# abacusorg/zeldovich-PLT

Hardware: AMD Instinct MI355X
Metric: particles/sec (grid->displacements) (higher is better)
Workload: dtype f64

## Files before the change

### zeldovich_plt_amd/api.py

```python
import ctypes as C
import os

import numpy as np

_HERE = os.path.dirname(os.path.abspath(__file__))
LIB_PATH = os.environ.get("ZD_LIB_PATH") or os.path.join(_HERE, "csrc", "build", "libzeldovich_hip.so")

ICFORMATS = {"Zeldovich": 0, "RVZel": 1, "RVdoubleZel": 2, "ZelSimple": 3}
RECORD_DTYPES = {
    "Zeldovich": np.dtype([("ijk", "<u2", 3), ("pad", "<u2"), ("d", "<f8", 3)]),
    "RVZel": np.dtype([("ijk", "<u2", 3), ("pad", "<u2"), ("d", "<f4", 3), ("v", "<f4", 3)]),
    "RVdoubleZel": np.dtype([("ijk", "<u2", 3), ("pad", "<u2"), ("d", "<f8", 3), ("v", "<f8", 3)]),
    "ZelSimple": np.dtype([("d", "<f4", 3)]),
}
KERNEL_NAMES = ("k_gen", "k_zfft", "k_yfft", "k_xfft", "z_stage", "exchange_wait")


class ZdParams(C.Structure):
    _fields_ = [
        ("ppd", C.c_int64), ("numblock", C.c_int32), ("cpd", C.c_int32), ("boxsize", C.c_double),
        ("fundamental", C.c_double), ("nyquist", C.c_double), ("k_cutoff", C.c_double),
        ("f_cluster", C.c_double), ("z_initial", C.c_double), ("PLT_target_z", C.c_double),
        ("seed", C.c_int64), ("corner_modes", C.c_int32), ("qdensity", C.c_int32),
        ("qoneslab", C.c_int32), ("qonemode", C.c_int32), ("one_mode", C.c_int32 * 3),
# ... 47 lines not shown
PASS_CB = C.CFUNCTYPE(C.c_int, C.c_void_p, C.c_int, C.c_int64, C.c_int64, C.c_void_p, C.c_void_p)
PARTICLE_CB = C.CFUNCTYPE(C.c_int, C.c_void_p, C.c_int64, C.c_int64, C.c_void_p)

EXPORTED_SYMBOLS = [
    "zd_generate", "zd_choose_stream_factor", "zd_plan_create", "zd_plan_destroy", "zd_plan_narray", "zd_plan_store_mode",
    "zd_plan_stream_factor", "zd_plan_passes", "zd_plan_plane_step", "zd_plan_record_size", "zd_plan_exchange_bytes", "zd_plan_local_planes",
    "zd_plan_plane_z", "zd_plan_stage_z", "zd_plan_stage_y", "zd_plan_stage_x", "zd_plan_stats", "zd_comm_unique_id", "zd_comm_create", "zd_comm_destroy", "zd_plan_ring_bytes", "zd_plan_run_pass",
    "zd_params_from_file", "zd_pk_create_from_file", "zd_pk_create_powerlaw", "zd_pk_power",
    "zd_pk_sigmaR", "zd_pk_destroy", "zd_load_eigmodes", "zd_free", "zd_comm_abort", "zd_comm_traffic", "zd_choose_pass_groups", "zd_plan_run_passes", "zd_comm_probe", "zd_choose_pass_groups_measured",
    "zd_dispatch_report", "zd_power_nbins", "zd_plan_measure_power", "zd_measure_power",
    "zd_plan_direct_sum", "zd_direct_sum", "zd_make_eigenmodes", "zd_write_eigmodes", "zd_param_file_string",
    "zd_plan_lpt_direct_sum", "zd_lpt_direct_sum", "zd_plan_lpt_power", "zd_lpt_power",
    "zd_interp_create", "zd_interp_add_plane", "zd_interp_result", "zd_interp_destroy", "zd_plan_interp", "zd_displace",
]
TESTING_SYMBOLS = ["zd_test_draws", "zd_test_modes", "zd_test_modes_table", "zd_test_v1_words", "zd_test_generate_loopback", "zd_test_fail_rank",
                   "zd_test_fft", "zd_test_ycols", "zd_test_poison", "zd_test_route", "zd_test_route_kernels", "zd_test_lpt2_coefficients", "zd_test_live_handles", "zd_test_plt_matrix"]
STORE_MODES = {"auto": 0, "reference": 1, "packed": 2, "fields": 3}

_lib = None
_testing_lib = None
TESTING_LIB_PATH = os.environ.get("ZD_TESTING_LIB_PATH") or os.path.join(_HERE, "csrc", "build", "libzeldovich_hip_testing.so")


def load_library():
    global _lib
    if _lib is None:
        _lib = _load(LIB_PATH, testing=False)
    return _lib


def load_testing_library():
# ... 13 lines not shown
    except ImportError:
        pass
    L = C.CDLL(path)
    vp, i32, i64, dbl = C.c_void_p, C.c_int32, C.c_int64, C.c_double
    L.zd_generate.argtypes = [C.POINTER(ZdParams), C.POINTER(ZdPk), vp, i64, SLAB_CB, vp, C.POINTER(ZdStats)]
    if testing:
        L.zd_test_generate_loopback.argtypes = L.zd_generate.argtypes
        L.zd_test_draws.argtypes = [i64, i64, vp, vp]
        L.zd_test_modes.argtypes = [C.POINTER(ZdParams), C.POINTER(ZdPk), i64, vp, vp]
        L.zd_test_modes_table.argtypes = [C.POINTER(ZdParams), C.POINTER(ZdPk), i64, vp, vp]
        L.zd_test_v1_words.argtypes = [i64, C.c_int32, vp]
        L.zd_test_fft.argtypes = [i32, i64, i32, vp, vp]
        L.zd_test_ycols.argtypes = [i32, i32, i32, i32, i32, vp, vp]
        L.zd_test_poison.argtypes = [C.c_int]
        L.zd_test_poison.restype = None
        L.zd_test_lpt2_coefficients.argtypes = [C.POINTER(ZdParams), vp]
        L.zd_test_lpt2_coefficients.restype = None
        L.zd_test_live_handles.argtypes = []
        L.zd_test_live_handles.restype = i64
        L.zd_test_plt_matrix.argtypes = [i64, dbl, i32, i64, vp, vp]
        L.zd_test_route_kernels.argtypes = [C.POINTER(ZdParams), i32, i32, i32, C.c_char_p, i64]
    L.zd_choose_stream_factor.argtypes = [C.POINTER(ZdParams), C.c_int, i64]
    L.zd_choose_pass_groups.argtypes = [C.POINTER(ZdParams), C.c_int, i64, C.POINTER(i32), C.POINTER(i32)]
    L.zd_plan_create.argtypes = [C.POINTER(ZdParams), C.POINTER(ZdPk), vp, i64, C.c_int, C.c_int, C.POINTER(vp)]
    L.zd_plan_destroy.argtypes = [vp]
    L.zd_plan_destroy.restype = None
    for name in ("zd_plan_narray", "zd_plan_store_mode", "zd_plan_stream_factor", "zd_plan_record_size", "zd_plan_passes", "zd_plan_plane_step"):
        getattr(L, name).argtypes = [vp]
        getattr(L, name).restype = i32
    for name in ("zd_plan_exchange_bytes", "zd_plan_local_planes"):
# ... 670 lines not shown
```

### zeldovich_plt_amd/csrc/zd_capi.cpp

```cpp
#include <hip/hip_runtime.h>

#include <atomic>
#include <chrono>
#include <condition_variable>
#include <deque>
#include <functional>
#include <mutex>
#include <new>
#include <thread>
#include <cmath>
#include <cstdio>
#include <cstdlib>
#include <cstring>
#include <vector>

#include "../../include/zeldovich_hip.h"
#include "zd_device.h"
#include "zd_launch.h"
#include "zd_plan.h"
#include "zd_glass.h"
#include "zd_route.h"
#include "zd_plt.h"
#ifdef ZD_TUNING
#include "zd_tuning.h"
// ... 46 lines not shown
            line[n - 1] = '\n';
        }
        if (buf && w == need && w + n < cap) {
            memcpy(buf + w, line, (size_t) n);
            w += n;
        }
        need += n;
    }
    if (buf && cap > 0) buf[w] = 0;
    return need + 1;
}

#ifdef ZD_TESTING
static std::atomic<int> g_poison{0};
void zd_test_poison(int on) { g_poison.store(on); }
#endif
hipError_t zd_store_alloc(void **p, size_t bytes) {
    hipError_t e = hipMalloc(p, bytes);
#ifdef ZD_TESTING
    if (e == hipSuccess && g_poison.load()) e = hipMemset(*p, 0xFF, bytes);
#endif
    return e;
}

namespace {

std::vector<cplx> make_twiddles(int n) {
    std::vector<cplx> tw(n);
    for (int k = 0; k < n; k++) {
        const long double a = 2.0L * 3.14159265358979323846264338327950288L * (long double) k / (long double) n;
// ... 921 lines not shown
                lBk = a; lBz = b; S.rows_outer = o;
            }
        }
        const int max_lBk = S.lHq + 1;
        while (lBk > max_lBk) lBk--;
        while ((1 << lBz) > pl->Zq) lBz--;
        S.lBk = lBk;
        S.lBz = lBz;
        S.one_block = (pl->nranks == 1 && lBk == S.lHq + 1 && lBz == 0 && !S.rows_outer) ? 1 : 0;
        int row_pad = store_row_pad(pl->N);
        if (const char *env = tune_env("ZD_PAD")) sscanf(env, "%d", &row_pad);
        pl->fused_z = pl->pack == zd::PACK_PLT3 && p->store_mode == ZD_STORE_AUTO && S.one_block && zd::genz_plt_supported(pl->N, pl->L)
                      && g.genf_tab && !v1 && p->qoneslab < 0 && main && p->k_cutoff >= 1.0
                      && (g.kmax == pl->half || !p->corner_modes) && (S.prune & 7) == 7 && !tune_env("ZD_NO_FUSED_Z");
        S.lq         = pl->fused_z ? 2 : 0;
        if (S.lq && !tune_env("ZD_PAD")) row_pad = store_row_pad(pl->N) / 2;
        S.pitch      = (pl->N + row_pad) << S.lq;
        S.a_rows     = (1 << lBk) << lBz;
        S.zb_rows    = S.a_rows * pl->narray;
        S.kb_rows    = S.zb_rows * ((pl->Zq >> S.lq) >> lBz);
        S.chunk_rows = S.kb_rows * ((2 * pl->Hq) >> lBk);
    }

    pl->ec.N        = pl->N;
    pl->ec.narray   = pl->narray;
    pl->ec.icformat = p->icformat;
    pl->ec.recsize  = record_size(p->icformat);
    pl->ec.qPLT     = p->qPLT;
    pl->ec.qdensity = p->qdensity;
    pl->ec.vnorm    = (p->qPLT || p->q2LPT) ? 1.0 : (sqrt(1. + 24 * p->f_cluster) - 1) * .25;
// ... 66 lines not shown
    zd::StoreLayout &S = pl->S;
    std::vector<zd::FieldRow> rows;
    const int64_t fe = field_rows(&pl->p, pl->nranks, &rows);
    HIPCHECK(upload(pl->d_fieldrows, rows));
    pl->F.lG          = S.lG;
    pl->F.lZq         = 0;
    while ((1 << pl->F.lZq) < pl->Zq) pl->F.lZq++;
    pl->F.Zq          = pl->Zq;
    pl->F.field_elems = fe;
    pl->F.ndens       = pl->dens ? 2 : 0;
    pl->F.nfield      = pl->pack == zd::PACK_PLTFIELD ? 6 : 4 + pl->F.ndens;
    pl->F.chunk_elems = (int64_t) pl->Zq * pl->F.nfield * fe;
    pl->F.rows        = pl->d_fieldrows;
    pl->store_bytes_  = pl->F.chunk_elems * pl->nranks * 16;
    pl->ring_planes = field_ring_planes(pl->N, pl->Zq);
    zd::StoreLayout &Q = pl->SR;
    Q            = S;
    Q.lq         = 0;
    Q.Hq         = pl->half;
    Q.lHq        = 0;
    while ((1 << Q.lHq) < pl->half) Q.lHq++;
    Q.lG         = 0;
    Q.ky_stride  = 1;
    Q.narray     = 3;
    Q.lBk        = Q.lHq + 1;
    Q.lBz        = 0;
    Q.rows_outer = 0;
    Q.one_block  = 1;
    Q.prune      = 0;
    Q.pitch      = pl->N + store_row_pad(pl->N);
// ... 1164 lines not shown
    zd::StoreLayout S;
    S.N = n; S.half = n / 2; S.Hq = n / 2; S.narray = narray;
    S.lHq = 0;
    while ((1 << S.lHq) < S.Hq) S.lHq++;
    S.lG = 0;
    S.ky_stride = 1;
    int lBk = 0, lBz = 0;
    if (tiled) {
        const long long target = std::max<long long>(1, ((long long) 2 << 20) / ((long long) n * 16));
        int lt = 0;
        while ((1LL << (lt + 1)) <= target) lt++;
        lBk = (lt + 1) / 2; lBz = lt - lBk;
        while ((1 << lBz) > nplanes) lBz--;
    }
    S.lq = 0;
    S.lBk = lBk; S.lBz = lBz; S.rows_outer = 0; S.one_block = 0; S.pitch = n; S.prune = 0; S.nt = 0; S.kmax = 0; S.fund2 = 0; S.k2_cutoff = 0;
    S.a_rows = (1 << lBk) << lBz;
    S.zb_rows = S.a_rows * narray;
    S.kb_rows = S.zb_rows * (nplanes >> lBz);
    S.chunk_rows = S.kb_rows * (n >> lBk);
    const size_t nel = (size_t) S.chunk_rows * S.pitch;
    DevBuf<cplx> d_tw, d;
    if (upload(d_tw, make_twiddles(n)) != hipSuccess || d.alloc(nel) != hipSuccess || hipMemset(d, 0, nel * sizeof(cplx)) != hipSuccess) return 1;
    float ms = 0;
    if (time_launches(reps, [&] { return zd::launch_yfft_variant(variant, S, nplanes, d_tw, d, 0); }, &ms)) return 1;
    *ms_per_launch = ms / reps;
    return 0;
}

int zd_test_copy_bw(int64_t bytes, int32_t reps, double *gbps) {
// ... 12 lines not shown
```

### zeldovich_plt_amd/csrc/zd_device.h

```cpp
#pragma once
#include <stdint.h>
#include "zd_fft.h"
#include "zd_pcg.h"
#if !defined(__HIPCC__)
struct double2 { double x, y; };
#endif

#ifdef ZD_TUNING
#define ZD_TUNE(x) ((x) != 0)
#else
#define ZD_TUNE(x) (false)
#endif

namespace zd {

constexpr int PK_LUT = 2048;

struct GenConst {
    int N, half;
    int kmax;
    int corner_modes;
    int qonemode, one_mode[3];
    int ablate;
    double fundamental, fundamental2, k2_cutoff;
// ... 55 lines not shown

struct StoreLayout {
    int N, half, Hq, narray;
    int lHq;
    int lG;
    int ky_stride;
    int lBk, lBz;
    int rows_outer;
    int one_block;
    int pitch;
    int chunk_rows, kb_rows, zb_rows, a_rows;
    int prune, kmax;
    double fund2, k2_cutoff;
    int nt;
    int lq;
};

constexpr int PRUNE_YTILE = 1 << 15;

ZD_HD bool column_is_zero(const StoreLayout &L, int kx, int ky) {
    if (!L.prune) return false;
    const int ax = kx < 0 ? -kx : kx, ay = ky < 0 ? -ky : ky;
    if (ax == L.kmax || ay == L.kmax) return true;
    return L.k2_cutoff > 0 && (double) (kx * kx + ky * ky) * L.fund2 >= L.k2_cutoff;
}

ZD_HD void row_slot(const StoreLayout &L, int ky, int &chunk, int &slot) {
    int kyh, tw;
    if (ky < L.half) {
        kyh = ky;
        tw  = 0;
// ... 104 lines not shown
ZD_HD void any_chunk_row(const AnyChunks &C, int y, int &chunk, int &slot) {
    const int half = C.N / 2;
    const int h = y < half ? y : (y == half ? 0 : C.N - y), tw = y < half ? 0 : 1;
    chunk = h & (C.G - 1);
    slot  = h / C.G + tw * C.Hq;
}

constexpr int NSLOT = 64;
struct Reduce {
    double sumsq[NSLOT];
    unsigned long long maxabs[3][NSLOT];
    unsigned long long maxkey[3][NSLOT];
    unsigned int lock[NSLOT];
};

template <int NT, int W>
__device__ __forceinline__ void ytile_of(int id, int &tile, int &a) {
    constexpr int TPL = W >= 8 ? 1 : 8 / W, GS = 6 * TPL;
    if constexpr (NT % (16 * TPL) == 0) {
        const int xcd = id & 7, s = id >> 3;
        const int g = (s / GS) * 8 + xcd, m = s % GS;
        const int side = m / (3 * TPL), mm = m % (3 * TPL);
        a    = mm / TPL;
        tile = side ? NT - 1 - (TPL * g + mm % TPL) : TPL * g + mm % TPL;
    } else {
        tile = id % NT;
        a    = id / NT;
    }
}

#if defined(__HIPCC__)
__device__ __forceinline__ bool mode_is_zero(const GenConst &g, int kx, int ky, int kz, double k2) {
    const int ax = kx < 0 ? -kx : kx, ay = ky < 0 ? -ky : ky, az = kz < 0 ? -kz : kz;
    if (ax == g.kmax || az == g.kmax || ay == g.kmax) return true;
// ... 8 lines not shown
```

### zeldovich_plt_amd/csrc/zd_kernels.hip

```cpp
#include <hip/hip_runtime.h>
#include <type_traits>
#include <stdint.h>
#include <stdio.h>
#include <algorithm>
#include <type_traits>
#include <stdlib.h>

#include "zd_device.h"
#include "zd_epi.h"
#include "zd_launch.h"
#include "zd_genmath.h"

using namespace zd;
using zdfft::cplx;
using zdpcg::u128;
using namespace zdgen;

__constant__ zdpcg::BitTable c_bits;

typedef double zd_d2v __attribute__((ext_vector_type(2)));
__device__ __forceinline__ cplx ld_stream(const cplx *p, bool nt) {
    if (nt) {
        const zd_d2v q = __builtin_nontemporal_load(reinterpret_cast<const zd_d2v *>(p));
        return cplx{q.x, q.y};
// ... 1204 lines not shown
    zdfft::fft_line<PL, LDS>(re, im, t, w, lds, twL);
    const FieldRow row = F.rows[kyloc0 / FIELD_RB + grp];
    const unsigned pos = ((unsigned) (x < row.split ? x : x - row.gap)) * FIELD_RB + r;
    const int Zq = 1 << F.lZq;
    int t2 = t;
    asm volatile("" : "+v"(t2));
#pragma unroll
    for (int e = 0; e < E; e++) {
        const int z2  = t2 + T * e;
        const int dst = z2 >> F.lZq, zl = z2 & (Zq - 1);
        out[(long long) dst * F.chunk_elems + (long long) (zl * F.nfield + (int) blockIdx.z) * F.field_elems + (unsigned) row.base + pos]
            = cplx{re[e], im[e]};
    }
}

template <int N, int E, int W, bool TWO>
__device__ __forceinline__ void yfft_f_unit_t(const FieldLayout &F, const StoreLayout &S, const cplx *__restrict__ tw,
                                              const cplx *__restrict__ store, int plane0, int ring_pitch, cplx *__restrict__ ring,
                                              int tile, int a, int pz, int unit, int t, int w, double *lds);

template <int N, int E, int W>
__device__ __forceinline__ void yfft_f_unit(const FieldLayout &F, const StoreLayout &S, const cplx *__restrict__ tw,
                                            const cplx *__restrict__ store, int plane0, int ring_pitch, cplx *__restrict__ ring,
                                            int id, int pz, int t, int w, double *lds) {
    using PL  = zdfft::Plan<N, E>;
    using LDS = zdfft::ColsInner<N, W>;
    constexpr int T = PL::T;
    constexpr int NT = N / W;
    int tile, a;
    ytile_of<NT, W>(id, tile, a);
    const int unit = pz * 3 * NT + id;
    if (F.nfield == 6 || a == 2)
        yfft_f_unit_t<N, E, W, true>(F, S, tw, store, plane0, ring_pitch, ring, tile, a, pz, unit, t, w, lds);
    else
        yfft_f_unit_t<N, E, W, false>(F, S, tw, store, plane0, ring_pitch, ring, tile, a, pz, unit, t, w, lds);
}

template <int N, int E, int W, bool TWO>
__device__ __forceinline__ void yfft_f_unit_t(const FieldLayout &F, const StoreLayout &S, const cplx *__restrict__ tw,
                                              const cplx *__restrict__ store, int plane0, int ring_pitch, cplx *__restrict__ ring,
                                              int tile, int a, int pz, [[maybe_unused]] int unit, int t, int w, double *lds) {
    using PL  = zdfft::Plan<N, E>;
    using LDS = zdfft::ColsInner<N, W>;
    constexpr int T = PL::T;
    const int x = tile * W + w, xm = (N - x) & (N - 1);
    const int zl = plane0 + pz;
#ifdef ZD_STAMPS
    if (zd_stamps && threadIdx.x == 0) {
        zd_stamps[(size_t) unit * 8 + 6] = __builtin_amdgcn_s_memrealtime();
        zd_stamps[(size_t) unit * 8 + 7] = (unsigned long long) __builtin_amdgcn_s_getreg((4 << 0) | (0 << 6) | (31 << 11))
                                           | ((unsigned long long) __builtin_amdgcn_s_getreg((20 << 0) | (0 << 6) | (31 << 11)) << 32);
    }
#endif
    ZD_STAMP(0, unit, false);
    const int kx = x > N / 2 ? x - N : x;
    if ((S.prune & PRUNE_YTILE) && __syncthreads_and(column_is_zero(S, kx, 0))) return;
    const bool plt = F.nfield == 6;
    constexpr bool two = TWO;
    const int f0 = plt ? (a == 0 ? 0 : (a == 1 ? 1 : 4)) : (a == 2 ? 1 : 2 * a);
    const int f1 = plt ? (a == 0 ? 3 : (a == 1 ? 2 : 5)) : 3;
    const cplx *p0 = store + (long long) (zl * F.nfield + f0) * F.field_elems;
    const long long d01 = two ? (long long) (f1 - f0) * F.field_elems : 0;
    const int gmask = (1 << F.lG) - 1;
    double re[E], im[E];
    FieldRow *rtab = reinterpret_cast<FieldRow *>(lds + LDS::SIZE);
    const int nblk = (S.Hq + FIELD_RB - 1) / FIELD_RB;
    for (int i = threadIdx.x; i < nblk; i += W * T) rtab[i] = F.rows[i];
    zdfft::TwSet<PL> twp;
    zdfft::load_twiddles<PL>(twp, t, tw);
    unsigned skipm = 1u << ((N / 2 - t) / T);
    if (t != 0) skipm = 0;
    if (S.prune & 4) {
        int c2 = 0x7fffffff;
        if (S.k2_cutoff > 0) {
            int m = (int) (S.k2_cutoff / S.fund2);
            while (m > 0 && (double) m * S.fund2 >= S.k2_cutoff) m--;
            while ((double) m * S.fund2 < S.k2_cutoff) m++;
            c2 = m;
        }
        const int akx = kx < 0 ? -kx : kx, kx2 = kx * kx;
#pragma unroll
        for (int e = 0; e < E; e++) {
            const int y = t + T * e, kyp = y > N / 2 ? N - y : y;
            if (akx == S.kmax || kyp == S.kmax || kx2 + kyp * kyp >= c2) skipm |= 1u << e;
        }
    }
// ... 27 lines not shown
        const cplx *p1 = p0 + d01;
#pragma unroll
        for (int b = 0; b < E; b += HB) {
            cplx v[HB];
            int tb = t;
            asm volatile("" : "+v"(tb));
#pragma unroll
            for (int j = 0; j < HB; j++) v[j] = p1[locate(tb, b + j)];
            asm volatile("" : "+v"(tb));
#pragma unroll
            for (int j = 0; j < HB; j++) {
                const int e = b + j, y = tb + T * e;
                const double s = y > N / 2 ? -1.0 : 1.0;
                const double ur = re[e], ui = im[e];
                const bool skip = (skipm >> e) & 1u;
                re[e] = skip ? 0.0 : -ui - s * v[j].x;
                im[e] = skip ? 0.0 : s * ur - v[j].y;
            }
        }
    } else {
        const double dkx = (double) kx;
        int tc = t;
        asm volatile("" : "+v"(tc));
#pragma unroll
        for (int e = 0; e < E; e++) {
            const int y = tc + T * e;
            const bool mir = y > N / 2;
            const double s = mir ? -1.0 : 1.0, dky = (double) (mir ? N - y : y);
            const double ur = re[e], ui = im[e];
            const bool skip = (skipm >> e) & 1u;
            re[e] = skip ? 0.0 : -s * (dky * ur + dkx * ui);
            im[e] = skip ? 0.0 : dkx * ur - dky * ui;
        }
    }
    if (ZD_TUNE(S.prune & 4096) && a == 2) return;
    ZD_STAMP(2, unit, true);
    if (!ZD_TUNE(S.prune & 128)) zdfft::fft_line_tw<PL, LDS>(re, im, t, w, lds, tw, twp);
    ZD_STAMP(3, unit, false);
    if (ZD_TUNE(S.prune & 256) && re[0] != 123.456) return;
    char *base = reinterpret_cast<char *>(ring + ((long long) (pz * 3 + a) * N) * ring_pitch);
    const unsigned xb = (unsigned) x * 16u, pb = (unsigned) ring_pitch * 16u;
    int t2 = t;
    asm volatile("" : "+v"(t2));
#pragma unroll
    for (int e = 0; e < E; e++) {
        const int y = t2 + T * e;
        const unsigned slot = y < N / 2 ? y : (y == N / 2 ? N / 2 : N / 2 + (N - y));
        if constexpr (N > 8192)
            *reinterpret_cast<cplx *>(base + ((size_t) slot * pb + xb)) = cplx{re[e], im[e]};
        else
            st_stream(reinterpret_cast<cplx *>(base + (slot * pb + xb)), cplx{re[e], im[e]}, ZD_NTBIT(S, 32));
    }
    ZD_STAMP(4, unit, false);
    ZD_STAMP(5, unit, true);
}
template <int N, int E, int W, int MINW = 1>
__global__ __launch_bounds__(W *N / E, MINW) void k_yfft_f(FieldLayout F, StoreLayout S, const cplx *__restrict__ tw,
                                                          const cplx *__restrict__ store, int plane0, int ring_pitch,
                                                          cplx *__restrict__ ring) {
    extern __shared__ __attribute__((aligned(16))) double lds[];
    yfft_f_unit<N, E, W>(F, S, tw, store, plane0, ring_pitch, ring, (int) blockIdx.x, (int) blockIdx.z, (int) threadIdx.x / W,
                         (int) threadIdx.x % W, lds);
}
template <int N, int E, int W, int MINW = 1>
__global__ __launch_bounds__(W *N / E, MINW) void k_yfft_fp(FieldLayout F, StoreLayout S, const cplx *__restrict__ tw,
                                                           const cplx *__restrict__ store, int plane0, int ring_pitch,
                                                           cplx *__restrict__ ring, int nplanes) {
    extern __shared__ __attribute__((aligned(16))) double lds[];
    constexpr int PER = 3 * (N / W);
    const int nwork = PER * nplanes;
#pragma unroll 1
    for (int work = blockIdx.x; work < nwork; work += gridDim.x) {
        int tid = threadIdx.x;
        asm volatile("" : "+v"(tid));
        yfft_f_unit<N, E, W>(F, S, tw, store, plane0, ring_pitch, ring, work % PER, work / PER, tid / W, tid % W, lds);
    }
}

constexpr int XFFT_NH(int N, int NA, int ROWS) {
    int nh = 1;
    while ((long long) ROWS * 2 * NA * N * 8 / nh > 65536 && nh < 16) nh *= 2;
    return nh;
}

constexpr int XFFT_SEQ_NH(int N, int NA, int lds_dbl) {
    int nh = 1;
    while (2 * NA * (N / nh) > lds_dbl && nh < 16) nh *= 2;
    return nh;
}

// ... 164 lines not shown
            fld[(row * 2 * NA + 2 * a) * NXH + xl]     = re[e];
            fld[(row * 2 * NA + 2 * a + 1) * NXH + xl] = im[e];
        }
        __syncthreads();
        xfft_consume<N, NA, ROWS, NXH, NT>(ec, fld, h, z, plane_rec0, records, density, ssq, mx);
    }
#pragma unroll
    for (int j = 0; j < 3; j++) {
        const unsigned lt = (unsigned) mx.tag[j], w2 = lt / (unsigned) (ROWS * N), rr = (lt / (unsigned) N) % (unsigned) ROWS, xx = lt % (unsigned) N;
        mg.v[j]   = mx.v[j];
        mg.lin[j] = ((unsigned long long) (z + (int) w2 * ec.z_pair) * N + (unsigned long long) (blockIdx.x * ROWS + rr)) * N + xx;
    }
    xfft_reduce<NT, NA>(lds, red, ssq, mg);
}

template <int N, int E>
__global__ __launch_bounds__(N / E, 2) void k_xfft_seq(StoreLayout S, EpiConst ec, const cplx *__restrict__ tw,
                                                   const cplx *__restrict__ data, int plane0, int z_first, int z_step,
                                                   char *__restrict__ records, Reduce *__restrict__ red) {
    using PL  = zdfft::Plan<N, E>;
    using LDS = zdfft::LineInner<N, 1>;
    extern __shared__ __attribute__((aligned(16))) double lds[];
    constexpr int T = PL::T, NT = T;
    const int t = threadIdx.x;
    const int y = blockIdx.x, pl = plane0 + blockIdx.y;
    double *czi = lds + LDS::SIZE;
    double cr[E];
#pragma unroll
    for (int e = 0; e < E; e++) cr[e] = 0.0;
    const int z = z_first + z_step * (int) blockIdx.y;
    MaxAbs mx;
    const long long plane_rec0 = 2 * (long long) blockIdx.y * N * N;
#pragma unroll 1
    for (int it = 0; it < 3; it++) {
        const int a = it == 0 ? 2 : it - 1;
        const cplx *src = data + row_offset(S, pl, a, y);
        double re[E], im[E];
        int ta = t;
        asm volatile("" : "+v"(ta));
#pragma unroll
        for (int e = 0; e < E; e++) {
            const cplx v = src[x_is_dead(ec, ta + T * e) ? 0 : ta + T * e];
            re[e] = v.x;
            im[e] = v.y;
        }
        int t3 = t;
        asm volatile("" : "+v"(t3));
#pragma unroll
        for (int e = 0; e < E; e++)
            if (x_is_dead(ec, t3 + T * e)) re[e] = im[e] = 0.0;
        __syncthreads();
        zdfft::fft_line<PL, LDS>(re, im, t, 0, lds, tw);
        int t2 = t;
        asm volatile("" : "+v"(t2));
        if (it == 0) {
#pragma unroll
            for (int e = 0; e < E; e++) {
                cr[e] = re[e];
                czi[t2 + T * e] = im[e];
            }
            continue;
        }
#pragma unroll
        for (int e = 0; e < E; e++) {
            const int xx = t2 + T * e;
            const double pos[3] = {re[e], im[e], a ? czi[xx] : cr[e]};
// ... 748 lines not shown
#endif
    switch (L) {
        ZCASE(32, 16, 4)
        ZCASE(64, 16, 4)
        ZCASE(128, 16, 4)
        ZCASE(256, 16, 2)
        ZCASE(512, 16, 1)
        ZCASE(1024, 16, 1)
        ZCASE(2048, 16, 1)
    }
#undef ZCASE
    ZD_TABLE_MISS("zeldovich_hip: field store: unsupported z-FFT length %d (power of two in [32,2048] required)\n", L);
    return 2;
}

template <int N, int E, int W, bool PERSIST = false, int MINW = 1>
static int launch_yfft_f_t(const FieldLayout &F, const StoreLayout &S, const void *tw, const void *store, int plane0,
                           int nplanes, int ring_pitch, void *ring, hipStream_t st) {
    constexpr int threads = W * N / E;
    const size_t shmem = sizeof(double) * (zdfft::ColsInner<N, W>::SIZE + (size_t) ((S.Hq + FIELD_RB - 1) / FIELD_RB));
    const size_t shmem_max = std::min<size_t>(160 * 1024, sizeof(double) * (zdfft::ColsInner<N, W>::SIZE + (size_t) (N / 2 + FIELD_RB - 1) / FIELD_RB));
    if (shmem > 160 * 1024) {
        ZD_TABLE_MISS("zeldovich_hip: y stage of the field store needs %zu B of LDS at PPD %d\n", shmem, N);
        return 2;
    }
    ZD_PROBE_RETURN();
    if constexpr (PERSIST) {
        set_dyn_lds<k_yfft_fp<N, E, W, MINW>>(shmem_max);
        int dev = 0, ncu = 256;
        hipGetDevice(&dev);
        hipDeviceGetAttribute(&ncu, hipDeviceAttributeMultiprocessorCount, dev);
        const int per_cu = std::max(1, std::min((int) (160 * 1024 / shmem), 2048 / (threads * (MINW > 1 ? 1 : 2))));
        dim3 grid((unsigned) std::max(8, ncu * per_cu / 8 * 8)), block(threads);
        hipLaunchKernelGGL((k_yfft_fp<N, E, W, MINW>), grid, block, shmem, st, F, S, (const cplx *) tw, (const cplx *) store, plane0,
                           ring_pitch, (cplx *) ring, nplanes);
        ZD_LAUNCH_CHECK();
    } else {
        set_dyn_lds<k_yfft_f<N, E, W, MINW>>(shmem_max);
        dim3 grid(3 * (N / W), 1, nplanes), block(threads);
        hipLaunchKernelGGL((k_yfft_f<N, E, W, MINW>), grid, block, shmem, st, F, S, (const cplx *) tw, (const cplx *) store, plane0,
                           ring_pitch, (cplx *) ring);
    }
    ZD_LAUNCH_CHECK();
    return 0;
}
int launch_yfft_fields(const FieldLayout &F, const StoreLayout &S, const void *tw, const void *store, int plane0,
                       int nplanes, int ring_pitch, void *ring, hipStream_t st) {
#define YCASE(n, e, w) \
    case n: return launch_yfft_f_t<n, e, w>(F, S, tw, store, plane0, nplanes, ring_pitch, ring, st);
#ifdef ZD_TUNING
    {
        const int yw = getenv("ZD_YW") ? atoi(getenv("ZD_YW")) : 0, yp = getenv("ZD_YPERSIST") ? atoi(getenv("ZD_YPERSIST")) : 0;
        if (S.N == 4096 && yw == 2 && !yp) return launch_yfft_f_t<4096, 16, 2, false, 4>(F, S, tw, store, plane0, nplanes, ring_pitch, ring, st);
        if (S.N == 4096 && yw == 2 && yp) return launch_yfft_f_t<4096, 16, 2, true, 4>(F, S, tw, store, plane0, nplanes, ring_pitch, ring, st);
        if (S.N == 4096 && yp) return launch_yfft_f_t<4096, 16, 4, true>(F, S, tw, store, plane0, nplanes, ring_pitch, ring, st);
        if (S.N == 2048 && yw == 4 && !yp) return launch_yfft_f_t<2048, 16, 4, false, 4>(F, S, tw, store, plane0, nplanes, ring_pitch, ring, st);
        if (S.N == 2048 && yw == 4 && yp) return launch_yfft_f_t<2048, 16, 4, true, 4>(F, S, tw, store, plane0, nplanes, ring_pitch, ring, st);
        if (S.N == 2048 && yp) return launch_yfft_f_t<2048, 16, 8, true>(F, S, tw, store, plane0, nplanes, ring_pitch, ring, st);
    }
#endif
    switch (S.N) {
        YCASE(64, 16, 32)
        YCASE(128, 16, 32)
        YCASE(256, 16, 16)
        YCASE(512, 16, 16)
        YCASE(1024, 16, 8)
// ... 47 lines not shown
    if constexpr (NA == 3) {
        if (ec.pack == PACK_PLT3) {
            set_dyn_lds<k_xfft<N, E, NA, ROWS, true>>(shmem);
            hipLaunchKernelGGL((k_xfft<N, E, NA, ROWS, true>), grid, block, shmem, st, S, ec, (const cplx *) tw, (const cplx *) data, plane0,
                               z_first, z_step, (char *) records, density, red);
            ZD_LAUNCH_CHECK();
            return 0;
        }
    }
    set_dyn_lds<k_xfft<N, E, NA, ROWS>>(shmem);
    hipLaunchKernelGGL((k_xfft<N, E, NA, ROWS>), grid, block, shmem, st, S, ec, (const cplx *) tw, (const cplx *) data,
                       plane0, z_first, z_step, (char *) records, density, red);
    ZD_LAUNCH_CHECK();
    return 0;
}
template <int N, int E>
static int launch_xfft_seq_t(const StoreLayout &S, const EpiConst &ec, const void *tw, const void *data, int plane0,
                             int nplanes, int z_first, int z_step, void *records, Reduce *red, hipStream_t st) {
    const size_t shmem = sizeof(double) * (zdfft::LineInner<N, 1>::SIZE + N);
    ZD_PROBE_RETURN();
    set_dyn_lds<k_xfft_seq<N, E>>(shmem);
    dim3 grid(N, nplanes), block(N / E);
    hipLaunchKernelGGL((k_xfft_seq<N, E>), grid, block, shmem, st, S, ec, (const cplx *) tw, (const cplx *) data, plane0, z_first,
                       z_step, (char *) records, red);
    ZD_LAUNCH_CHECK();
    return 0;
}

template <int N, int E, bool SPLIT2 = false>
static int launch_xfft_seq_plt_t(const StoreLayout &S, const EpiConst &ec, const void *tw, const void *data, int plane0,
                                 int nplanes, int z_first, int z_step, void *records, Reduce *red, hipStream_t st) {
    const size_t shmem = sizeof(double) * (zdfft::LineInner<N, 1>::SIZE + (SPLIT2 ? 1 : 2) * N);
    ZD_PROBE_RETURN();
    set_dyn_lds<k_xfft_seq_plt<N, E, SPLIT2>>(shmem);
    dim3 grid(N, nplanes), block(N / E);
    hipLaunchKernelGGL((k_xfft_seq_plt<N, E, SPLIT2>), grid, block, shmem, st, S, ec, (const cplx *) tw, (const cplx *) data, plane0, z_first,
                       z_step, (char *) records, red);
    ZD_LAUNCH_CHECK();
// ... 31 lines not shown
template <int N, int E, bool PLT>
static int launch_xfft_two_t(const StoreLayout &S, const EpiConst &ec, const void *tw, const void *data, int plane0,
                             int nplanes, int z_first, int z_step, void *records, Reduce *red, hipStream_t st) {
    const size_t shmem = sizeof(double) * zdfft::LineInner<N, 1>::SIZE;
    ZD_PROBE_RETURN();
    set_dyn_lds<k_xfft_two<N, E, PLT>>(shmem);
    for (int emit = 0; emit < 2; emit++) {
        dim3 grid(N, nplanes, (emit != 0) == PLT ? 1 : 2), block(N / E);
        hipLaunchKernelGGL((k_xfft_two<N, E, PLT>), grid, block, shmem, st, S, ec, (const cplx *) tw, (cplx *) data, emit, plane0, z_first,
                           z_step, (char *) records, red);
        ZD_LAUNCH_CHECK();
    }
    return 0;
}

int launch_xfft(const StoreLayout &S, const EpiConst &ec, const void *tw, const void *data, int plane0, int nplanes,
                int z_first, int z_step, void *records, float *density, Reduce *red, hipStream_t st) {
    if (S.lq) {
        if (S.lq == 2 && S.one_block && S.narray == 3 && ec.pack == PACK_PLT3 && !density) {
            if (S.N == 2048) return launch_xfft_q2_plt_t<2048, 16>(S, ec, tw, data, plane0, nplanes, z_first, z_step, records, red, st);
            if (S.N == 1024) return launch_xfft_q2_plt_t<1024, 16>(S, ec, tw, data, plane0, nplanes, z_first, z_step, records, red, st);
            if (S.N == 512) return launch_xfft_q2_plt_t<512, 16>(S, ec, tw, data, plane0, nplanes, z_first, z_step, records, red, st);
        }
        ZD_TABLE_MISS("zeldovich_hip: no x pass for plane-interleaved rows at PPD %d\n", S.N);
        return 2;
    }
    if (S.N == 8192 && S.narray == 3 && ec.pack == PACK_ZAFIELD)
        return launch_xfft_seq_t<8192, 16>(S, ec, tw, data, plane0, nplanes, z_first, z_step, records, red, st);
    if (S.N == 4096 && S.narray == 3 && ec.pack == PACK_ZAFIELD)
        return launch_xfft_seq_t<4096, 16>(S, ec, tw, data, plane0, nplanes, z_first, z_step, records, red, st);
    if (S.N == 1024 && S.narray == 3 && ec.pack == PACK_ZAFIELD)
        return launch_xfft_seq_t<1024, 16>(S, ec, tw, data, plane0, nplanes, z_first, z_step, records, red, st);
    if (S.N == 2048 && S.narray == 3 && ec.pack == PACK_ZAFIELD)
        return launch_xfft_seq_t<2048, 16>(S, ec, tw, data, plane0, nplanes, z_first, z_step, records, red, st);
    if (S.N == 16384 && S.narray == 3 && ec.pack == PACK_ZAFIELD)
        return launch_xfft_two_t<16384, 16, false>(S, ec, tw, data, plane0, nplanes, z_first, z_step, records, red, st);
    if (S.N == 8192 && S.narray == 3 && ec.pack == PACK_PLT3)
        return launch_xfft_two_t<8192, 16, true>(S, ec, tw, data, plane0, nplanes, z_first, z_step, records, red, st);
    if (S.N == 4096 && S.narray == 3 && ec.pack == PACK_PLT3)
        return launch_xfft_seq_plt_t<4096, 16, true>(S, ec, tw, data, plane0, nplanes, z_first, z_step, records, red, st);

    if (S.N == 2048 && S.narray == 3 && ec.pack == PACK_PLT3)
        return launch_xfft_seq_plt_t<2048, 16, true>(S, ec, tw, data, plane0, nplanes, z_first, z_step, records, red, st);
#define XCASE(n, e, rows1, rows2, rows4, rows3z, rows3p)                                                              \
    case n:                                                                                                           \
        if (S.narray == 1) return launch_xfft_t<n, e, 1, rows1>(S, ec, tw, data, plane0, nplanes, z_first, z_step, records, density, red, st); \
        if (S.narray == 2) return launch_xfft_t<n, e, 2, rows2>(S, ec, tw, data, plane0, nplanes, z_first, z_step, records, density, red, st); \
        if (S.narray == 3 && ec.pack == PACK_ZAPAIR)                                                                  \
            return launch_xfft_t<n, e, 3, rows3z>(S, ec, tw, data, plane0, nplanes, z_first, z_step, records, density, red, st); \
// ... 150 lines not shown
```

### zeldovich_plt_amd/csrc/zd_tables.h

```cpp
#pragma once
#include "zd_device.h"
#include "zd_launch.h"

namespace zd {

inline bool has_zfft(int L) {
    TableProbe probe;
    const JobList jobs{};
    const StoreLayout S{};
    return launch_zfft(L, jobs, S, 0, 0, 1, 1, nullptr, nullptr, nullptr, nullptr) == 0;
}
inline bool has_zfft_fields(int L, int nky) {
    TableProbe probe;
    const FieldLayout F{};
    const StoreLayout S{};
    return launch_zfft_fields(L, F, S, 0, 0, nky, nullptr, nullptr, nullptr, nullptr) == 0;
}
inline bool has_yfft(int N, int lq, int one_block, int nplanes) {
    TableProbe probe;
    StoreLayout S{};
    S.N         = N;
    S.lq        = lq;
    S.one_block = one_block;
    S.pitch     = (N + (lq ? (N >= 512 ? 12 : 0) : (N >= 512 ? 24 : 0))) << lq;
// ... 2 lines not shown
inline bool has_yfft_fields(int N, int Hq) {
    TableProbe probe;
    const FieldLayout F{};
    StoreLayout S{};
    S.N  = N;
    S.Hq = Hq;
    return launch_yfft_fields(F, S, nullptr, nullptr, 0, 1, 0, nullptr, nullptr) == 0;
}
inline bool has_xfft(int N, int narray, int pack, int lq, int one_block) {
    TableProbe probe;
    StoreLayout S{};
    S.N         = N;
    S.narray    = narray;
    S.lq        = lq;
    S.one_block = one_block;
    EpiConst ec{};
    ec.N      = N;
    ec.narray = narray;
    ec.pack   = pack;
    return launch_xfft(S, ec, nullptr, nullptr, 0, 1, 0, 1, nullptr, nullptr, nullptr, nullptr) == 0;
}
inline bool has_fnl_stage(int N) {
    TableProbe probe;
    StoreLayout S{};
    S.N = N;
    return launch_fnl_stage(0, S, 0., nullptr, nullptr, nullptr, 1, 0, nullptr) == 0;
}
inline bool has_lpt2_xsrc(int N) {
    TableProbe probe;
    StoreLayout S{};
// ... 91 lines not shown
```

### zeldovich_plt_amd/csrc/zd_testing.h

```cpp
#pragma once
#include "../../include/zeldovich_hip.h"
#ifdef __cplusplus
extern "C" {
#endif
#pragma GCC visibility push(default)
int zd_test_route(const zd_params *p, int32_t R, int32_t nranks, int32_t *out, char *why, int64_t cap);
int zd_test_route_kernels(const zd_params *p, int32_t R, int32_t nranks, int32_t role, char *text, int64_t cap);
void zd_test_lpt2_coefficients(const zd_params *p, double *out);
int64_t zd_test_live_handles(void);
int zd_test_draws(int64_t seed, int64_t n, const int32_t *kxyz, uint64_t *out);
int zd_test_modes(const zd_params *p, const zd_pk *pk, int64_t n, const int32_t *kxyz, double *D);
int zd_test_modes_table(const zd_params *p, const zd_pk *pk, int64_t n, const int32_t *kxyz, double *out);
int zd_test_generate_loopback(const zd_params *p, const zd_pk *pk, const double *eig, int64_t eig_ppd, zd_slab_cb cb, void *user,
                              zd_stats *out);
int zd_test_v1_words(int64_t seed, int32_t nblocks, uint32_t *out);
int zd_test_fft(int32_t n, int64_t lines, int32_t axis_kind, const double *in, double *out);
int zd_test_ycols(int32_t n, int32_t G, int32_t ncols, int32_t nimg, int32_t mode, const double *in, double *out);
void zd_test_poison(int on);
void zd_test_fail_rank(int rank);
int zd_test_plt_matrix(int64_t n, double alpha, int32_t shells, int64_t nmodes, const int32_t *m_xyz, double *out6);
#pragma GCC visibility pop
#ifdef __cplusplus
}
#endif
```

Measured before the change: 31.69 billion.

## Pair mirrored kx columns in y-FFT ring tiles for ZA field path

For the 4-field ZA pack at N=1024/2048/4096, y-FFT tiles now cover paired columns x and N-x together, using conjugate symmetry so mirrored lines reuse the same loaded data, and write them adjacently into the ring. The x-FFT pass then permutes ring rows back to natural order through LDS before its line FFT, and applies dead-x masking through the column mapping. This aims to cut store reads and improve locality in the y stage. In exchange the x pass gains two extra LDS scatter/gather rounds with syncs, and the tile-to-XCD mapping changes.

Result: faster. 32.07 billion, median of 6 (+1.2%).

```diff
diff --git a/zeldovich_plt_amd/api.py b/zeldovich_plt_amd/api.py
--- a/zeldovich_plt_amd/api.py
+++ b/zeldovich_plt_amd/api.py
@@ -85,7 +85,8 @@
     "zd_interp_create", "zd_interp_add_plane", "zd_interp_result", "zd_interp_destroy", "zd_plan_interp", "zd_displace",
 ]
 TESTING_SYMBOLS = ["zd_test_draws", "zd_test_modes", "zd_test_modes_table", "zd_test_v1_words", "zd_test_generate_loopback", "zd_test_fail_rank",
-                   "zd_test_fft", "zd_test_ycols", "zd_test_poison", "zd_test_route", "zd_test_route_kernels", "zd_test_lpt2_coefficients", "zd_test_live_handles", "zd_test_plt_matrix"]
+                   "zd_test_fft", "zd_test_ycols", "zd_test_poison", "zd_test_route", "zd_test_route_kernels", "zd_test_lpt2_coefficients", "zd_test_live_handles", "zd_test_plt_matrix",
+                   "zd_test_ring_pair_w"]
 STORE_MODES = {"auto": 0, "reference": 1, "packed": 2, "fields": 3}
 
 _lib = None
@@ -129,6 +130,8 @@
         L.zd_test_ycols.argtypes = [i32, i32, i32, i32, i32, vp, vp]
         L.zd_test_poison.argtypes = [C.c_int]
         L.zd_test_poison.restype = None
+        L.zd_test_ring_pair_w.argtypes = [C.c_int]
+        L.zd_test_ring_pair_w.restype = None
         L.zd_test_lpt2_coefficients.argtypes = [C.POINTER(ZdParams), vp]
         L.zd_test_lpt2_coefficients.restype = None
         L.zd_test_live_handles.argtypes = []
diff --git a/zeldovich_plt_amd/csrc/zd_capi.cpp b/zeldovich_plt_amd/csrc/zd_capi.cpp
--- a/zeldovich_plt_amd/csrc/zd_capi.cpp
+++ b/zeldovich_plt_amd/csrc/zd_capi.cpp
@@ -84,6 +84,8 @@
 #ifdef ZD_TESTING
 static std::atomic<int> g_poison{0};
 void zd_test_poison(int on) { g_poison.store(on); }
+static std::atomic<int> g_ring_pair_w{0};
+void zd_test_ring_pair_w(int w) { g_ring_pair_w.store(w); }
 #endif
 hipError_t zd_store_alloc(void **p, size_t bytes) {
     hipError_t e = hipMalloc(p, bytes);
@@ -1035,6 +1037,7 @@
                       && g.genf_tab && !v1 && p->qoneslab < 0 && main && p->k_cutoff >= 1.0
                       && (g.kmax == pl->half || !p->corner_modes) && (S.prune & 7) == 7 && !tune_env("ZD_NO_FUSED_Z");
         S.lq         = pl->fused_z ? 2 : 0;
+        S.paired     = 0;
         if (S.lq && !tune_env("ZD_PAD")) row_pad = store_row_pad(pl->N) / 2;
         S.pitch      = (pl->N + row_pad) << S.lq;
         S.a_rows     = (1 << lBk) << lBz;
@@ -1131,6 +1134,10 @@
     pl->F.rows        = pl->d_fieldrows;
     pl->store_bytes_  = pl->F.chunk_elems * pl->nranks * 16;
     pl->ring_planes = field_ring_planes(pl->N, pl->Zq);
+    S.paired = pl->pack == zd::PACK_ZAFIELD && pl->F.nfield == 4 ? zd::ring_pair_w(pl->N) : 0;
+#ifdef ZD_TESTING
+    if (S.paired && pl->N == 1024 && g_ring_pair_w.load() == 4) S.paired = 4;
+#endif
     zd::StoreLayout &Q = pl->SR;
     Q            = S;
     Q.lq         = 0;
@@ -2325,6 +2332,7 @@
         while ((1 << lBz) > nplanes) lBz--;
     }
     S.lq = 0;
+    S.paired = 0;
     S.lBk = lBk; S.lBz = lBz; S.rows_outer = 0; S.one_block = 0; S.pitch = n; S.prune = 0; S.nt = 0; S.kmax = 0; S.fund2 = 0; S.k2_cutoff = 0;
     S.a_rows = (1 << lBk) << lBz;
     S.zb_rows = S.a_rows * narray;
diff --git a/zeldovich_plt_amd/csrc/zd_device.h b/zeldovich_plt_amd/csrc/zd_device.h
--- a/zeldovich_plt_amd/csrc/zd_device.h
+++ b/zeldovich_plt_amd/csrc/zd_device.h
@@ -93,7 +93,20 @@
     double fund2, k2_cutoff;
     int nt;
     int lq;
-};
+    int paired;
+};
+
+constexpr int ring_pair_w(int N) { return N == 4096 ? 4 : (N == 2048 || N == 1024 ? 8 : 0); }
+ZD_HD int ring_pair_pos(int N, int W, int x) {
+    const int h = W >> 1, m = x < N / 2 ? x : (N - x) & (N / 2 - 1);
+    const int g2 = 2 * (m & ~(h - 1)), i = m & (h - 1);
+    return x < N / 2 ? g2 + i : g2 + W - 1 - i;
+}
+ZD_HD int ring_pair_col(int N, int W, int p) {
+    const int h = W >> 1, i = p & (W - 1), g = (p & ~(W - 1)) >> 1;
+    const int m = g + (i < h ? i : W - 1 - i);
+    return i < h ? m : (m ? N - m : N / 2);
+}
 
 constexpr int PRUNE_YTILE = 1 << 15;
 
@@ -228,10 +241,25 @@
     unsigned int lock[NSLOT];
 };
 
-template <int NT, int W>
+template <int NT, int W, bool PAIR = false>
 __device__ __forceinline__ void ytile_of(int id, int &tile, int &a) {
     constexpr int TPL = W >= 8 ? 1 : 8 / W, GS = 6 * TPL;
-    if constexpr (NT % (16 * TPL) == 0) {
+    if constexpr (PAIR) {
+        static_assert(NT % (8 * TPL) == 0, "paired y tiles: whole groups per XCD");
+#ifndef ZD_YPAIR_ORDER
+#define ZD_YPAIR_ORDER 0
+#endif
+        if constexpr (ZD_YPAIR_ORDER == 1) {
+            const int r = id % NT, xcd = r & 7, s = r >> 3;
+            a    = id / NT;
+            tile = TPL * ((s / TPL) * 8 + xcd) + s % TPL;
+        } else {
+            const int xcd = id & 7, s = id >> 3;
+            const int g = (s / (3 * TPL)) * 8 + xcd, m = s % (3 * TPL);
+            a    = m / TPL;
+            tile = TPL * g + m % TPL;
+        }
+    } else if constexpr (NT % (16 * TPL) == 0) {
         const int xcd = id & 7, s = id >> 3;
         const int g = (s / GS) * 8 + xcd, m = s % GS;
         const int side = m / (3 * TPL), mm = m % (3 * TPL);
diff --git a/zeldovich_plt_amd/csrc/zd_kernels.hip b/zeldovich_plt_amd/csrc/zd_kernels.hip
--- a/zeldovich_plt_amd/csrc/zd_kernels.hip
+++ b/zeldovich_plt_amd/csrc/zd_kernels.hip
@@ -1242,12 +1242,12 @@
     }
 }
 
-template <int N, int E, int W, bool TWO>
+template <int N, int E, int W, bool TWO, bool PAIR>
 __device__ __forceinline__ void yfft_f_unit_t(const FieldLayout &F, const StoreLayout &S, const cplx *__restrict__ tw,
                                               const cplx *__restrict__ store, int plane0, int ring_pitch, cplx *__restrict__ ring,
                                               int tile, int a, int pz, int unit, int t, int w, double *lds);
 
-template <int N, int E, int W>
+template <int N, int E, int W, bool PAIR>
 __device__ __forceinline__ void yfft_f_unit(const FieldLayout &F, const StoreLayout &S, const cplx *__restrict__ tw,
                                             const cplx *__restrict__ store, int plane0, int ring_pitch, cplx *__restrict__ ring,
                                             int id, int pz, int t, int w, double *lds) {
@@ -1256,22 +1256,24 @@
     constexpr int T = PL::T;
     constexpr int NT = N / W;
     int tile, a;
-    ytile_of<NT, W>(id, tile, a);
+    ytile_of<NT, W, PAIR>(id, tile, a);
     const int unit = pz * 3 * NT + id;
     if (F.nfield == 6 || a == 2)
-        yfft_f_unit_t<N, E, W, true>(F, S, tw, store, plane0, ring_pitch, ring, tile, a, pz, unit, t, w, lds);
+        yfft_f_unit_t<N, E, W, true, PAIR>(F, S, tw, store, plane0, ring_pitch, ring, tile, a, pz, unit, t, w, lds);
     else
-        yfft_f_unit_t<N, E, W, false>(F, S, tw, store, plane0, ring_pitch, ring, tile, a, pz, unit, t, w, lds);
-}
-
-template <int N, int E, int W, bool TWO>
+        yfft_f_unit_t<N, E, W, false, PAIR>(F, S, tw, store, plane0, ring_pitch, ring, tile, a, pz, unit, t, w, lds);
+}
+
+template <int N, int E, int W, bool TWO, bool PAIR>
 __device__ __forceinline__ void yfft_f_unit_t(const FieldLayout &F, const StoreLayout &S, const cplx *__restrict__ tw,
                                               const cplx *__restrict__ store, int plane0, int ring_pitch, cplx *__restrict__ ring,
                                               int tile, int a, int pz, [[maybe_unused]] int unit, int t, int w, double *lds) {
     using PL  = zdfft::Plan<N, E>;
     using LDS = zdfft::ColsInner<N, W>;
     constexpr int T = PL::T;
-    const int x = tile * W + w, xm = (N - x) & (N - 1);
+    static_assert(!PAIR || (W >= 2 && N / 2 % (W / 2) == 0), "paired tiles: whole half groups");
+    const bool dline = PAIR && w >= W / 2;
+    const int x = PAIR ? tile * (W / 2) + (dline ? W - 1 - w : w) : tile * W + w, xm = (N - x) & (N - 1);
     const int zl = plane0 + pz;
 #ifdef ZD_STAMPS
     if (zd_stamps && threadIdx.x == 0) {
@@ -1298,6 +1300,7 @@
     zdfft::load_twiddles<PL>(twp, t, tw);
     unsigned skipm = 1u << ((N / 2 - t) / T);
     if (t != 0) skipm = 0;
+    if (PAIR && dline && x == 0) skipm = (1u << E) - 1u;
     if (S.prune & 4) {
         int c2 = 0x7fffffff;
         if (S.k2_cutoff > 0) {
@@ -1355,8 +1358,14 @@
                 const double s = y > N / 2 ? -1.0 : 1.0;
                 const double ur = re[e], ui = im[e];
                 const bool skip = (skipm >> e) & 1u;
-                re[e] = skip ? 0.0 : -ui - s * v[j].x;
-                im[e] = skip ? 0.0 : s * ur - v[j].y;
+                if constexpr (PAIR) {
+                    const double vx = dline ? -v[j].x : v[j].x, vy = dline ? -v[j].y : v[j].y;
+                    re[e] = skip ? 0.0 : -ui - s * vx;
+                    im[e] = skip ? 0.0 : s * ur - vy;
+                } else {
+                    re[e] = skip ? 0.0 : -ui - s * v[j].x;
+                    im[e] = skip ? 0.0 : s * ur - v[j].y;
+                }
             }
         }
     } else {
@@ -1367,11 +1376,20 @@
         for (int e = 0; e < E; e++) {
             const int y = tc + T * e;
             const bool mir = y > N / 2;
-            const double s = mir ? -1.0 : 1.0, dky = (double) (mir ? N - y : y);
-            const double ur = re[e], ui = im[e];
-            const bool skip = (skipm >> e) & 1u;
-            re[e] = skip ? 0.0 : -s * (dky * ur + dkx * ui);
-            im[e] = skip ? 0.0 : dkx * ur - dky * ui;
+            if constexpr (PAIR) {
+                const int iky = mir ? N - y : y;
+                const double s = mir ? -1.0 : 1.0, dky = (double) (dline ? -iky : iky);
+                const double ur = re[e], ui = im[e];
+                const bool skip = (skipm >> e) & 1u;
+                re[e] = skip ? 0.0 : -s * (dky * ur + dkx * ui);
+                im[e] = skip ? 0.0 : dkx * ur - dky * ui;
+            } else {
+                const double s = mir ? -1.0 : 1.0, dky = (double) (mir ? N - y : y);
+                const double ur = re[e], ui = im[e];
+                const bool skip = (skipm >> e) & 1u;
+                re[e] = skip ? 0.0 : -s * (dky * ur + dkx * ui);
+                im[e] = skip ? 0.0 : dkx * ur - dky * ui;
+            }
         }
     }
     if (ZD_TUNE(S.prune & 4096) && a == 2) return;
@@ -1380,7 +1398,7 @@
     ZD_STAMP(3, unit, false);
     if (ZD_TUNE(S.prune & 256) && re[0] != 123.456) return;
     char *base = reinterpret_cast<char *>(ring + ((long long) (pz * 3 + a) * N) * ring_pitch);
-    const unsigned xb = (unsigned) x * 16u, pb = (unsigned) ring_pitch * 16u;
+    const unsigned xb = (unsigned) (PAIR ? tile * W + w : x) * 16u, pb = (unsigned) ring_pitch * 16u;
     int t2 = t;
     asm volatile("" : "+v"(t2));
 #pragma unroll
@@ -1390,20 +1408,20 @@
         if constexpr (N > 8192)
             *reinterpret_cast<cplx *>(base + ((size_t) slot * pb + xb)) = cplx{re[e], im[e]};
         else
-            st_stream(reinterpret_cast<cplx *>(base + (slot * pb + xb)), cplx{re[e], im[e]}, ZD_NTBIT(S, 32));
+            st_stream(reinterpret_cast<cplx *>(base + (slot * pb + xb)), cplx{re[e], (PAIR && dline) ? -im[e] : im[e]}, ZD_NTBIT(S, 32));
     }
     ZD_STAMP(4, unit, false);
     ZD_STAMP(5, unit, true);
 }
-template <int N, int E, int W, int MINW = 1>
+template <int N, int E, int W, int MINW = 1, bool PAIR = false>
 __global__ __launch_bounds__(W *N / E, MINW) void k_yfft_f(FieldLayout F, StoreLayout S, const cplx *__restrict__ tw,
                                                           const cplx *__restrict__ store, int plane0, int ring_pitch,
                                                           cplx *__restrict__ ring) {
     extern __shared__ __attribute__((aligned(16))) double lds[];
-    yfft_f_unit<N, E, W>(F, S, tw, store, plane0, ring_pitch, ring, (int) blockIdx.x, (int) blockIdx.z, (int) threadIdx.x / W,
+    yfft_f_unit<N, E, W, PAIR>(F, S, tw, store, plane0, ring_pitch, ring, (int) blockIdx.x, (int) blockIdx.z, (int) threadIdx.x / W,
                          (int) threadIdx.x % W, lds);
 }
-template <int N, int E, int W, int MINW = 1>
+template <int N, int E, int W, int MINW = 1, bool PAIR = false>
 __global__ __launch_bounds__(W *N / E, MINW) void k_yfft_fp(FieldLayout F, StoreLayout S, const cplx *__restrict__ tw,
                                                            const cplx *__restrict__ store, int plane0, int ring_pitch,
                                                            cplx *__restrict__ ring, int nplanes) {
@@ -1414,7 +1432,7 @@
     for (int work = blockIdx.x; work < nwork; work += gridDim.x) {
         int tid = threadIdx.x;
         asm volatile("" : "+v"(tid));
-        yfft_f_unit<N, E, W>(F, S, tw, store, plane0, ring_pitch, ring, work % PER, work / PER, tid / W, tid % W, lds);
+        yfft_f_unit<N, E, W, PAIR>(F, S, tw, store, plane0, ring_pitch, ring, work % PER, work / PER, tid / W, tid % W, lds);
     }
 }
 
@@ -1609,7 +1627,7 @@
     xfft_reduce<NT, NA>(lds, red, ssq, mg);
 }
 
-template <int N, int E>
+template <int N, int E, int PW = 0>
 __global__ __launch_bounds__(N / E, 2) void k_xfft_seq(StoreLayout S, EpiConst ec, const cplx *__restrict__ tw,
                                                    const cplx *__restrict__ data, int plane0, int z_first, int z_step,
                                                    char *__restrict__ records, Reduce *__restrict__ red) {
@@ -1635,7 +1653,8 @@
         asm volatile("" : "+v"(ta));
 #pragma unroll
         for (int e = 0; e < E; e++) {
-            const cplx v = src[x_is_dead(ec, ta + T * e) ? 0 : ta + T * e];
+            const int xe = PW ? ring_pair_col(N, PW, ta + T * e) : ta + T * e;
+            const cplx v = src[x_is_dead(ec, xe) ? 0 : ta + T * e];
             re[e] = v.x;
             im[e] = v.y;
         }
@@ -1643,8 +1662,24 @@
         asm volatile("" : "+v"(t3));
 #pragma unroll
         for (int e = 0; e < E; e++)
-            if (x_is_dead(ec, t3 + T * e)) re[e] = im[e] = 0.0;
+            if (x_is_dead(ec, PW ? ring_pair_col(N, PW, t3 + T * e) : t3 + T * e)) re[e] = im[e] = 0.0;
         __syncthreads();
+        if constexpr (PW != 0) {
+            int tb = t;
+            asm volatile("" : "+v"(tb));
+#pragma unroll
+            for (int e = 0; e < E; e++) lds[LDS::idx(ring_pair_col(N, PW, tb + T * e), 0)] = re[e];
+            __syncthreads();
+            zdfft::xchg_read<PL, LDS>(re, t, 0, lds);
+            __syncthreads();
+            int tc = t;
+            asm volatile("" : "+v"(tc));
+#pragma unroll
+            for (int e = 0; e < E; e++) lds[LDS::idx(ring_pair_col(N, PW, tc + T * e), 0)] = im[e];
+            __syncthreads();
+            zdfft::xchg_read<PL, LDS>(im, t, 0, lds);
+            __syncthreads();
+        }
         zdfft::fft_line<PL, LDS>(re, im, t, 0, lds, tw);
         int t2 = t;
         asm volatile("" : "+v"(t2));
@@ -2423,7 +2458,7 @@
     return 2;
 }
 
-template <int N, int E, int W, bool PERSIST = false, int MINW = 1>
+template <int N, int E, int W, bool PERSIST = false, int MINW = 1, bool PAIR = false>
 static int launch_yfft_f_t(const FieldLayout &F, const StoreLayout &S, const void *tw, const void *store, int plane0,
                            int nplanes, int ring_pitch, void *ring, hipStream_t st) {
     constexpr int threads = W * N / E;
@@ -2435,19 +2470,19 @@
     }
     ZD_PROBE_RETURN();
     if constexpr (PERSIST) {
-        set_dyn_lds<k_yfft_fp<N, E, W, MINW>>(shmem_max);
+        set_dyn_lds<k_yfft_fp<N, E, W, MINW, PAIR>>(shmem_max);
         int dev = 0, ncu = 256;
         hipGetDevice(&dev);
         hipDeviceGetAttribute(&ncu, hipDeviceAttributeMultiprocessorCount, dev);
         const int per_cu = std::max(1, std::min((int) (160 * 1024 / shmem), 2048 / (threads * (MINW > 1 ? 1 : 2))));
         dim3 grid((unsigned) std::max(8, ncu * per_cu / 8 * 8)), block(threads);
-        hipLaunchKernelGGL((k_yfft_fp<N, E, W, MINW>), grid, block, shmem, st, F, S, (const cplx *) tw, (const cplx *) store, plane0,
+        hipLaunchKernelGGL((k_yfft_fp<N, E, W, MINW, PAIR>), grid, block, shmem, st, F, S, (const cplx *) tw, (const cplx *) store, plane0,
                            ring_pitch, (cplx *) ring, nplanes);
         ZD_LAUNCH_CHECK();
     } else {
-        set_dyn_lds<k_yfft_f<N, E, W, MINW>>(shmem_max);
+        set_dyn_lds<k_yfft_f<N, E, W, MINW, PAIR>>(shmem_max);
         dim3 grid(3 * (N / W), 1, nplanes), block(threads);
-        hipLaunchKernelGGL((k_yfft_f<N, E, W, MINW>), grid, block, shmem, st, F, S, (const cplx *) tw, (const cplx *) store, plane0,
+        hipLaunchKernelGGL((k_yfft_f<N, E, W, MINW, PAIR>), grid, block, shmem, st, F, S, (const cplx *) tw, (const cplx *) store, plane0,
                            ring_pitch, (cplx *) ring);
     }
     ZD_LAUNCH_CHECK();
@@ -2455,10 +2490,21 @@
 }
 int launch_yfft_fields(const FieldLayout &F, const StoreLayout &S, const void *tw, const void *store, int plane0,
                        int nplanes, int ring_pitch, void *ring, hipStream_t st) {
-#define YCASE(n, e, w) \
-    case n: return launch_yfft_f_t<n, e, w>(F, S, tw, store, plane0, nplanes, ring_pitch, ring, st);
+#define YCASE(n, e, w)                                                                                                               \
+    case n:                                                                                                                          \
+        if constexpr (ring_pair_w(n) == w)                                                                                           \
+            if (S.paired == w) return launch_yfft_f_t<n, e, w, false, 1, true>(F, S, tw, store, plane0, nplanes, ring_pitch, ring, st); \
+        return launch_yfft_f_t<n, e, w>(F, S, tw, store, plane0, nplanes, ring_pitch, ring, st);
+    if (S.paired && (F.nfield != 4 || S.paired != ring_pair_w(S.N))) {
+#ifdef ZD_TESTING
+        if (F.nfield == 4 && S.N == 1024 && S.paired == 4)
+            return launch_yfft_f_t<1024, 16, 4, false, 1, true>(F, S, tw, store, plane0, nplanes, ring_pitch, ring, st);
+#endif
+        ZD_TABLE_MISS("zeldovich_hip: no y stage for paired ring rows of %d at PPD %d\n", S.paired, S.N);
+        return 2;
+    }
 #ifdef ZD_TUNING
-    {
+    if (!S.paired) {
         const int yw = getenv("ZD_YW") ? atoi(getenv("ZD_YW")) : 0, yp = getenv("ZD_YPERSIST") ? atoi(getenv("ZD_YPERSIST")) : 0;
         if (S.N == 4096 && yw == 2 && !yp) return launch_yfft_f_t<4096, 16, 2, false, 4>(F, S, tw, store, plane0, nplanes, ring_pitch, ring, st);
         if (S.N == 4096 && yw == 2 && yp) return launch_yfft_f_t<4096, 16, 2, true, 4>(F, S, tw, store, plane0, nplanes, ring_pitch, ring, st);
@@ -2536,14 +2582,14 @@
     ZD_LAUNCH_CHECK();
     return 0;
 }
-template <int N, int E>
+template <int N, int E, int PW = 0>
 static int launch_xfft_seq_t(const StoreLayout &S, const EpiConst &ec, const void *tw, const void *data, int plane0,
                              int nplanes, int z_first, int z_step, void *records, Reduce *red, hipStream_t st) {
     const size_t shmem = sizeof(double) * (zdfft::LineInner<N, 1>::SIZE + N);
     ZD_PROBE_RETURN();
-    set_dyn_lds<k_xfft_seq<N, E>>(shmem);
+    set_dyn_lds<k_xfft_seq<N, E, PW>>(shmem);
     dim3 grid(N, nplanes), block(N / E);
-    hipLaunchKernelGGL((k_xfft_seq<N, E>), grid, block, shmem, st, S, ec, (const cplx *) tw, (const cplx *) data, plane0, z_first,
+    hipLaunchKernelGGL((k_xfft_seq<N, E, PW>), grid, block, shmem, st, S, ec, (const cplx *) tw, (const cplx *) data, plane0, z_first,
                        z_step, (char *) records, red);
     ZD_LAUNCH_CHECK();
     return 0;
@@ -2605,6 +2651,19 @@
     return 0;
 }
 
+template <int N>
+static int xfft_seq_ring(const StoreLayout &S, const EpiConst &ec, const void *tw, const void *data, int plane0, int nplanes, int z_first,
+                         int z_step, void *records, Reduce *red, hipStream_t st) {
+    if (S.paired == ring_pair_w(N))
+        return launch_xfft_seq_t<N, 16, ring_pair_w(N)>(S, ec, tw, data, plane0, nplanes, z_first, z_step, records, red, st);
+#ifdef ZD_TESTING
+    if constexpr (N == 1024)
+        if (S.paired == 4) return launch_xfft_seq_t<N, 16, 4>(S, ec, tw, data, plane0, nplanes, z_first, z_step, records, red, st);
+#endif
+    ZD_TABLE_MISS("zeldovich_hip: no x pass for ring rows paired by %d at PPD %d\n", S.paired, N);
+    return 2;
+}
+
 int launch_xfft(const StoreLayout &S, const EpiConst &ec, const void *tw, const void *data, int plane0, int nplanes,
                 int z_first, int z_step, void *records, float *density, Reduce *red, hipStream_t st) {
     if (S.lq) {
@@ -2619,11 +2678,11 @@
     if (S.N == 8192 && S.narray == 3 && ec.pack == PACK_ZAFIELD)
         return launch_xfft_seq_t<8192, 16>(S, ec, tw, data, plane0, nplanes, z_first, z_step, records, red, st);
     if (S.N == 4096 && S.narray == 3 && ec.pack == PACK_ZAFIELD)
-        return launch_xfft_seq_t<4096, 16>(S, ec, tw, data, plane0, nplanes, z_first, z_step, records, red, st);
+        return xfft_seq_ring<4096>(S, ec, tw, data, plane0, nplanes, z_first, z_step, records, red, st);
     if (S.N == 1024 && S.narray == 3 && ec.pack == PACK_ZAFIELD)
-        return launch_xfft_seq_t<1024, 16>(S, ec, tw, data, plane0, nplanes, z_first, z_step, records, red, st);
+        return xfft_seq_ring<1024>(S, ec, tw, data, plane0, nplanes, z_first, z_step, records, red, st);
     if (S.N == 2048 && S.narray == 3 && ec.pack == PACK_ZAFIELD)
-        return launch_xfft_seq_t<2048, 16>(S, ec, tw, data, plane0, nplanes, z_first, z_step, records, red, st);
+        return xfft_seq_ring<2048>(S, ec, tw, data, plane0, nplanes, z_first, z_step, records, red, st);
     if (S.N == 16384 && S.narray == 3 && ec.pack == PACK_ZAFIELD)
         return launch_xfft_two_t<16384, 16, false>(S, ec, tw, data, plane0, nplanes, z_first, z_step, records, red, st);
     if (S.N == 8192 && S.narray == 3 && ec.pack == PACK_PLT3)
diff --git a/zeldovich_plt_amd/csrc/zd_tables.h b/zeldovich_plt_amd/csrc/zd_tables.h
--- a/zeldovich_plt_amd/csrc/zd_tables.h
+++ b/zeldovich_plt_amd/csrc/zd_tables.h
@@ -40,6 +40,7 @@
     S.narray    = narray;
     S.lq        = lq;
     S.one_block = one_block;
+    S.paired    = pack == PACK_ZAFIELD && narray == 3 ? ring_pair_w(N) : 0;
     EpiConst ec{};
     ec.N      = N;
     ec.narray = narray;
diff --git a/zeldovich_plt_amd/csrc/zd_testing.h b/zeldovich_plt_amd/csrc/zd_testing.h
--- a/zeldovich_plt_amd/csrc/zd_testing.h
+++ b/zeldovich_plt_amd/csrc/zd_testing.h
@@ -17,6 +17,7 @@
 int zd_test_fft(int32_t n, int64_t lines, int32_t axis_kind, const double *in, double *out);
 int zd_test_ycols(int32_t n, int32_t G, int32_t ncols, int32_t nimg, int32_t mode, const double *in, double *out);
 void zd_test_poison(int on);
+void zd_test_ring_pair_w(int w);
 void zd_test_fail_rank(int rank);
 int zd_test_plt_matrix(int64_t n, double alpha, int32_t shells, int64_t nmodes, const int32_t *m_xyz, double *out6);
 #pragma GCC visibility pop
```
